# 2thleZ/flash_attention_metal

Measured on AMD Instinct MI355X. Metric: attn_fwd_tflops (seqlen=4096, head_dim=64, bf16, causal), higher is better.
Workload: dtype bf16; 1 GPU; BASELINE.json configs[2]: seqlen=4096 head_dim=64 batch=4 heads=16 bf16 is_causal=true per GPU; batch_per_gpu=4, heads=16, seq_len=4096, head_dim=64, is_causal=True

## Files before the change

### flash_attention_metal_amd/csrc/fa_api.hip

```cpp
#include <stdarg.h>
#include <algorithm>
#include <initializer_list>
#include <stdio.h>
#include <string.h>

#include "fa_common.h"

namespace {
thread_local char g_err[512] = "";

int fail(int code, const char *fmt, ...) {
  va_list ap;
  va_start(ap, fmt);
  vsnprintf(g_err, sizeof(g_err), fmt, ap);
  va_end(ap);
  return code;
}

#define TRY(check) do { if (const int st_ = (check)) return st_; } while (0)

int nonnull(const char *fn, std::initializer_list<const void *> ptrs) {
  for (const void *p : ptrs)
    if (!p) return fail(FA_ERR_INVALID_ARG, "%s: null pointer", fn);
  return FA_OK;
// ... 84 lines not shown
  return e == hipSuccess ? FA_OK : fail(FA_ERR_LAUNCH, "%s: launch failed: %s", fn, hipGetErrorString(e));
}
}

extern "C" {

const char *fa_last_error(void) { return g_err; }
int fa_version(void) { return FA_MI355_VERSION; }

const char *fa_variant_name(int v) {
  switch (v) {
    case FA_VARIANT_AUTO: return "auto";
    case FA_VARIANT_NAIVE: return "naive";
    case FA_VARIANT_TILED: return "tiled";
    case FA_VARIANT_TILED_V2: return "tiled_v2";
    case FA_VARIANT_MFMA: return "mfma";
    case FA_VARIANT_MFMA_PP: return "mfma_pp";
    case FA_VARIANT_MFMA_SPLITKV: return "mfma_splitkv";
    case FA_VARIANT_MFMA_SPLIT2: return "mfma_split2";
    case FA_VARIANT_MFMA_EXACT: return "mfma_exact";
    case FA_VARIANT_MFMA_H64S2: return "mfma_h64s2";
    case FA_VARIANT_MFMA16: return "mfma16";
    case FA_VARIANT_MFMA_FP8PV: return "mfma_fp8pv";
    default: return "?";
  }
}
const char *fa_dtype_name(int d) {
  switch (d) {
    case FA_DTYPE_F32: return "f32";
    case FA_DTYPE_F16: return "f16";
    case FA_DTYPE_BF16: return "bf16";
    case FA_DTYPE_FP8_E4M3: return "fp8_e4m3";
    default: return "?";
  }
}
int fa_dtype_in_bytes(int d) {
  switch (d) {
    case FA_DTYPE_F32: return 4;
    case FA_DTYPE_F16: case FA_DTYPE_BF16: return 2;
    case FA_DTYPE_FP8_E4M3: return 1;
    default: return 0;
  }
}
int fa_dtype_out_bytes(int d) { return d == FA_DTYPE_FP8_E4M3 ? 2 : fa_dtype_in_bytes(d); }

int fa_supported(int dtype, int variant, int D) {
  switch (variant) {
    case FA_VARIANT_AUTO: return fa_resolve_variant(dtype, D) > 0;
    case FA_VARIANT_NAIVE: return fa::naive_supported(dtype, D);
    case FA_VARIANT_TILED: return fa::tiled_supported(dtype, D);
    case FA_VARIANT_TILED_V2: return fa::tiled_v2_supported(dtype, D);
    case FA_VARIANT_MFMA: return fa::mfma_supported(dtype, D);
    case FA_VARIANT_MFMA_PP: return 0;
    case FA_VARIANT_MFMA_SPLITKV: return fa::splitkv_supported(dtype, D);
    case FA_VARIANT_MFMA_SPLIT2: return fa::mfma_split2_supported(dtype, D);
    case FA_VARIANT_MFMA_EXACT: return fa::mfma_supported(dtype, D);
    case FA_VARIANT_MFMA_H64S2: return fa::mfma_h64s2_supported(dtype, D);
    case FA_VARIANT_MFMA16: return fa::mfma16_supported(dtype, D);
    case FA_VARIANT_MFMA_FP8PV: return fa::fp8pv_supported(dtype, D);
    default: return 0;
  }
}
int fa_resolve_variant(int dtype, int D) {
  if (fa::mfma_supported(dtype, D)) return FA_VARIANT_MFMA;
  if (fa::mfma16_supported(dtype, D)) return FA_VARIANT_MFMA16;
  if (fa::tiled_v2_supported(dtype, D)) return FA_VARIANT_TILED_V2;
  return FA_ERR_UNSUPPORTED;
}

static int route_auto(int dtype, int D, int B, int H, int Nq, int Nk, int is_causal, bool ex) {
  const long long blocks128 = (long long)B * H * ((Nq + 127) / 128);
  if (D == 64 && fa::splitkv_supported(dtype, D) && Nk > 64 && blocks128 <= 64) return FA_VARIANT_MFMA_SPLITKV;
  const int v = fa_resolve_variant(dtype, D);
  if (v != FA_VARIANT_MFMA) return v;
  if (ex)
    return fa::mfma16_supported(dtype, D) && blocks128 > 512 && Nk >= (D == 64 ? (is_causal ? 1536 : 1024) : (is_causal ? 2048 : 1024))
               ? FA_VARIANT_MFMA16
               : FA_VARIANT_MFMA;
  const int N = Nq;
  const long long blocks64 = (long long)B * H * ((N + 63) / 64);
  if (fa::mfma_h64s2_supported(dtype, D) && N >= 256 && blocks64 <= 512) return FA_VARIANT_MFMA_H64S2;
  const bool fp8_d128 = dtype == FA_DTYPE_FP8_E4M3 && D == 128;
// ... 42 lines not shown
double fa_algorithmic_bytes(int B, int H, int N, int D, int dtype) {
  return (3.0 * fa_dtype_in_bytes(dtype) + fa_dtype_out_bytes(dtype)) * (double)B * H * N * D +
         4.0 * (double)B * H * N;
}

static hipError_t launch_fwd(const void *q, const void *k, const void *v, void *o, float *lse, int B, int Hq, int Hkv, int Nq, int Nk,
                             int D, float scale, long long q_batch_stride, long long q_head_stride, long long kv_batch_stride,
                             long long kv_head_stride, int is_causal, int dtype, int variant, hipStream_t s) {
  fa::Params p;
  p.q = q; p.k = k; p.v = v; p.o = o; p.lse = lse;
  p.B = B; p.H = Hq; p.N = Nq; p.D = D; p.scale = scale;
  p.batch_stride = q_batch_stride; p.head_stride = q_head_stride;
  p.is_causal = is_causal ? 1 : 0;
  p.Nk = Nk; p.Hkv = Hkv; p.kv_batch_stride = kv_batch_stride; p.kv_head_stride = kv_head_stride;
  p.exact = (variant == FA_VARIANT_MFMA_EXACT);
  switch (variant) {
    case FA_VARIANT_NAIVE: return fa::launch_naive(p, dtype, s);
    case FA_VARIANT_TILED: return fa::launch_tiled(p, dtype, s);
    case FA_VARIANT_TILED_V2: return fa::launch_tiled_v2(p, dtype, s);
    case FA_VARIANT_MFMA_SPLITKV: return fa::launch_splitkv(p, dtype, s);
    case FA_VARIANT_MFMA_SPLIT2: return fa::launch_mfma_split2(p, dtype, s);
    case FA_VARIANT_MFMA_H64S2: return fa::launch_mfma_h64s2(p, dtype, s);
    case FA_VARIANT_MFMA16: return fa::launch_mfma16(p, dtype, s);
    case FA_VARIANT_MFMA_FP8PV: return fa::launch_fp8pv(p, dtype, s);
    default: return fa::launch_mfma(p, dtype, s);
  }
}

int fa_fwd(const void *q, const void *k, const void *v, void *o, float *lse, int B, int H, int N,
           int D, float scale, long long batch_stride, long long head_stride, int is_causal,
           int dtype, int variant, void *hip_stream) {
  g_err[0] = 0;
  const char *fn = "fa_fwd";
  TRY(nonnull(fn, {q, k, v, o}));
  TRY(positive(fn, {B, H, N, D}));
  TRY(scale_ok(fn, scale));
  if (fa_dtype_in_bytes(dtype) == 0) return fail(FA_ERR_INVALID_ARG, "fa_fwd: bad dtype %d", dtype);
  TRY(strides_ok(fn, "", N, D, batch_stride, head_stride, stride_mult(dtype), H > 1));
  TRY(aligned16(fn, "tensors", {q, k, v, o}));
  TRY(head_fits(fn, (double)(N + 128) * D * fa_dtype_in_bytes(dtype), 4, ""));
  if (!fa::mfma_supported(dtype, D) && fa::mfma16_supported(dtype, D))
    TRY(head_fits(fn, (double)(N + 128) * D * 2, 2, " (head dims on padded rows)"));
  TRY(grid_fits(fn, (long long)B * H, N));
  if (variant == FA_VARIANT_AUTO) {
    variant = route_auto(dtype, D, B, H, N, N, is_causal, false);
    if (variant < 0)
// ... 20 lines not shown
}

int fa_fwd_exv(const void *q, const void *k, const void *v, void *o, float *lse, int B, int Hq, int Hkv, int Nq, int Nk,
               int D, float scale, long long q_batch_stride, long long q_head_stride, long long kv_batch_stride,
               long long kv_head_stride, int is_causal, int dtype, int variant, void *hip_stream) {
  g_err[0] = 0;
  const char *fn = "fa_fwd_ex";
  TRY(nonnull(fn, {q, k, v, o}));
  TRY(positive(fn, {B, Hq, Hkv, Nq, Nk, D}));
  TRY(grouped(fn, Hq, Hkv));
  TRY(causal_fits(fn, is_causal, Nq, Nk));
  TRY(scale_ok(fn, scale));
  const bool padded_dim = !fa::mfma_supported(dtype, D) && fa::mfma16_supported(dtype, D);
  if (!fa::mfma_supported(dtype, D) && !padded_dim)
    return fail(FA_ERR_UNSUPPORTED, "fa_fwd_ex: needs a matrix-core kernel (f16/bf16: D a multiple of 8 up to 128, or 256; fp8: D=64|128|256), got dtype=%s D=%d",
                fa_dtype_name(dtype), D);
  if (padded_dim) TRY(head_fits(fn, (double)(std::max(Nq, Nk) + 128) * D * 2, 2, " (head dims on padded rows)"));
  TRY(strides_ok(fn, "", Nq, D, q_batch_stride, q_head_stride, stride_mult(dtype), Hq > 1 && B > 1));
  TRY(strides_ok(fn, "key/value ", Nk, D, kv_batch_stride, kv_head_stride, stride_mult(dtype), Hkv > 1 && B > 1));
  TRY(aligned16(fn, "tensors", {q, k, v, o}));
  TRY(head_fits(fn, (double)(std::max(Nq, Nk) + 128) * D * fa_dtype_in_bytes(dtype), 4, ""));
  TRY(grid_fits(fn, (long long)B * Hq, Nq));
  if (variant == FA_VARIANT_AUTO) variant = route_auto(dtype, D, B, Hq, Nq, Nk, is_causal, true);
  if (variant != FA_VARIANT_MFMA && variant != FA_VARIANT_MFMA_EXACT && variant != FA_VARIANT_MFMA16 && variant != FA_VARIANT_MFMA_SPLITKV)
    return fail(FA_ERR_UNSUPPORTED, "fa_fwd_ex: variant=%s does not take grouped heads / Nq != Nk (mfma, mfma_exact, mfma16, mfma_splitkv do)",
                fa_variant_name(variant));
  if (!fa_supported(dtype, variant, D))
    return fail(FA_ERR_UNSUPPORTED, "fa_fwd_ex: variant=%s does not support dtype=%s D=%d", fa_variant_name(variant), fa_dtype_name(dtype), D);
  return launched(fn, launch_fwd(q, k, v, o, lse, B, Hq, Hkv, Nq, Nk, D, scale, q_batch_stride, q_head_stride, kv_batch_stride,
                                 kv_head_stride, is_causal, dtype, variant, (hipStream_t)hip_stream));
}

int fa_fwd_varlen_supported(int dtype, int D) { return fa::mfma_varlen_supported(dtype, D); }
static int varlen_impl(const char *fn, const void *q, const void *k, const void *v, void *o, float *lse, const int *cu_seqlens_q,
                       const int *cu_seqlens_k, int B, int Hq, int Hkv, int total_q, int total_k, int max_seqlen_q, int max_seqlen_k, int D,
                       float scale, long long q_row_stride, long long q_head_stride, long long kv_row_stride, long long kv_head_stride,
                       int window_left, int window_right, int dtype, void *hip_stream, const float *const *sinks = nullptr,
                       const float *softcap = nullptr) {
  g_err[0] = 0;
  TRY(nonnull(fn, {q, k, v, o, cu_seqlens_q, cu_seqlens_k}));
  if (sinks) TRY(sinks_ok(fn, *sinks));
  if (softcap) TRY(softcap_ok(fn, *softcap));
  TRY(positive(fn, {B, Hq, Hkv, total_q, total_k, max_seqlen_q, max_seqlen_k, D}));
  TRY(grouped(fn, Hq, Hkv));
  TRY(scale_ok(fn, scale));
  if (!fa_fwd_varlen_supported(dtype, D))
    return fail(FA_ERR_UNSUPPORTED, "%s: needs f16 / bf16 and D = 64 | 128, got dtype=%s D=%d", fn, fa_dtype_name(dtype), D);
  if (max_seqlen_q > total_q || max_seqlen_k > total_k)
// ... 865 lines not shown
```

### flash_attention_metal_amd/csrc/fa_common.h

```cpp
#pragma once
#include <hip/hip_runtime.h>
#include <stdint.h>

#include <mutex>
#include <set>
#include <utility>

#include "../../include/fa_mi355.h"

namespace fa {

struct FastDiv {
  unsigned mul = 1, sh1 = 0, sh2 = 0;
};
inline FastDiv make_fastdiv(unsigned d) {
  unsigned l = 0;
  while ((1ull << l) < d) ++l;
  FastDiv f;
  f.mul = (unsigned)(((1ull << 32) * ((1ull << l) - d)) / d + 1);
  f.sh1 = l < 1 ? l : 1u;
  f.sh2 = l > 1 ? l - 1 : 0u;
  return f;
}

// ... 173 lines not shown
hipError_t launch_mfma_varlen_paged_sink(const VarlenPagedSinkParams &p, int dtype, hipStream_t s);
hipError_t launch_mfma_varlen_softcap(const VarlenSoftcapParams &p, int dtype, hipStream_t s);
hipError_t launch_mfma_varlen_paged_softcap(const VarlenPagedSoftcapParams &p, int dtype, hipStream_t s);
hipError_t launch_mfma_varlen_paged_kv8(const VarlenPagedSinkParams &p, bool with_sink, hipStream_t s);
bool mfma_varlen_paged_kv8_supported(int q_dtype, int kv_dtype, int D, int page_size);
hipError_t launch_mfma_varlen_paged_ksplit(const VarlenPagedKsplitParams &p, int dtype, hipStream_t s);
int varlen_paged_ksplit_splits(int B, int Hq, int max_seqlen_q, int D, int page_size, int max_pages_per_seq);
struct AppendPagedParams {
  const void *k_new, *v_new;
  void *k_pages, *v_pages;
  const int *cu_new, *block_table, *seqlens;
  int B, Hkv, total_new, max_new, D;
  long long new_rs, new_hs, page_stride, head_stride, row_stride;
  int bt_stride, num_pages, max_pages;
  int lp;
};
constexpr int APPEND_ROWS = 16;
hipError_t launch_kv_append_paged(const AppendPagedParams &p, int elem_bytes, hipStream_t s);
hipError_t launch_kv_append_paged_quant(const AppendPagedParams &p, int new_dtype, float k_mul, float v_mul, hipStream_t s);
hipError_t launch_mfma_split2(const Params &p, int dtype, hipStream_t s);
bool mfma_split2_supported(int dtype, int D);
hipError_t launch_mfma_h64s2(const Params &p, int dtype, hipStream_t s);
bool mfma_h64s2_supported(int dtype, int D);
hipError_t launch_mfma16(const Params &p, int dtype, hipStream_t s);
bool mfma16_supported(int dtype, int D);
int mfma16_waves(int D, int BH, int N, int Nk, int is_causal);
hipError_t launch_fp8pv(const Params &p, int dtype, hipStream_t s);
bool fp8pv_supported(int dtype, int D);
hipError_t launch_splitkv(const Params &p, int dtype, hipStream_t s);

hipError_t launch_decode(const DecodeParams &p, int D, int dtype, int kv8, hipStream_t s);
bool decode_supported(int dtype, int D);
int decode_splits(int B, int Hkv, int Nk, int D, int kv8);
long long decode_workspace_bytes(int B, int Hq, int Hkv, int Nq, int Nk, int D);
hipError_t launch_decode_paged(const DecodePagedParams &p, int D, int dtype, int kv8, hipStream_t s);
hipError_t launch_decode_paged_window(const DecodeWindowParams &p, int D, int dtype, int kv8, hipStream_t s);
hipError_t launch_decode_paged_sink(const DecodeWindowParams &p, const float *sinks, int D, int dtype, int kv8, hipStream_t s);
hipError_t launch_decode_paged_softcap(const DecodeSoftcapParams &p, int D, int dtype, int kv8, hipStream_t s);
hipError_t launch_mla_decode_paged(const MlaDecodeParams &p, int dtype, hipStream_t s);
bool mla_decode_supported(int dtype, int Dqk, int Dv);
int mla_decode_splits(int B, int rblk, int Nk);
long long mla_decode_workspace_bytes(int B, int Hq, int Nq, int Nk);
inline int mla_wide_waves(int rows) { return rows <= 32 ? 2 : 4; }
hipError_t launch_mla_decode_paged_wide(const MlaDecodeParams &p, int dtype, hipStream_t s);
hipError_t launch_mla_combine(const MlaDecodeParams &p, int dtype, hipStream_t s);
long long mla_decode_wide_workspace_bytes(int B, int Hq, int Nq, int Nk);
hipError_t launch_mla_decode_paged_kv8(const MlaDecodeParams &p, hipStream_t s);
long long mla_decode_kv8_workspace_bytes(int B, int Hq, int Nq, int Nk);
// ... 57 lines not shown
```

### flash_attention_metal_amd/csrc/fa_mfma16_kernel.hip

```cpp
#include <stdlib.h>

#include <algorithm>

#include "fa_mfma_common.h"

#ifndef FA16_DEFER_THR
#define FA16_DEFER_THR 8.0f
#endif
#ifndef FA16_LAK
#define FA16_LAK (D == 128 ? 3 : 2)
#endif
#ifndef FA16_LAV
#define FA16_LAV (D == 128 ? 3 : 2)
#endif
#ifndef FA16_PRIO
#define FA16_PRIO 1
#endif
#ifndef FA16_ONES
#define FA16_ONES 1
#endif
#ifndef FA16_LAZY
#define FA16_LAZY 1
#endif
#ifndef FA16_LAZY_THR
#define FA16_LAZY_THR 0x1p20f
// ... 24 lines not shown
#endif
#ifndef FA16_OCC
#define FA16_OCC 4
#endif

namespace fa {

typedef float f32x4 __attribute__((ext_vector_type(4)));

template <typename Tag> struct MT16;
template <> struct MT16<BF16> {
  using elem = __bf16;
  using vec8 = bf16x8;
  __device__ static __forceinline__ f32x4 mfma(vec8 a, vec8 b, f32x4 c) { return __builtin_amdgcn_mfma_f32_16x16x32_bf16(a, b, c, 0, 0, 0); }
};
template <> struct MT16<F16> {
  using elem = _Float16;
  using vec8 = f16x8;
  __device__ static __forceinline__ f32x4 mfma(vec8 a, vec8 b, f32x4 c) { return __builtin_amdgcn_mfma_f32_16x16x32_f16(a, b, c, 0, 0, 0); }
};

__device__ __forceinline__ float xlane(float x, int mask) { return __shfl_xor(x, mask, 64); }

template <typename Tag, int D, int SUB>
constexpr size_t mfma16_lds_bytes() {
  constexpr bool lazy = std::is_same<Tag, BF16>::value && D == 64 && (FA16_ONES != 0) && (FA16_LAZY == 1);
  return 4 * SUB * (size_t)(D == 128 ? FA16_BN128 : BN) * D * 2 + (lazy ? 16 : 0);
}

template <typename Tag, int D, bool CAUSAL, int RW, bool PAD, int SUB>
__device__ __forceinline__ void fwd_mfma16_body(const Params &p) {
  using M = MT16<Tag>;
  using vec8 = typename M::vec8;
  using elem = typename M::elem;
  constexpr int BMR = RW * WM;
  constexpr int RB = D * 2;
  constexpr int CPR = D / 8;
  constexpr int KS = D / 32;
  constexpr int DT = D / 16;
  constexpr int BNK = (D == 128) ? FA16_BN128 : BN;
  constexpr int KT = BNK / 16;
  constexpr int NKP = KT / 2;
  constexpr int TILE = BNK * RB;
  static_assert(D == 64 || D == 128, "head dims of the 16x16x32 kernel");

  extern __shared__ __attribute__((aligned(16))) char smem_generic[];
  lds_char *smem = (lds_char *)smem_generic;
  lds_char *Kbuf = smem;
  lds_char *Vbuf = smem + 2 * SUB * TILE;

  const int wave = __builtin_amdgcn_readfirstlane((int)threadIdx.x >> 6);
  const int lane = threadIdx.x & 63;
  const int c = lane & 15;
  const int g = lane >> 4;

  int bh, qb;
  map_block<CAUSAL>(blockIdx.x, p, bh, qb);
  long long base, base_kv;
  head_bases(bh, p, base, base_kv);
  const int coff = p.Nk - p.N;
  const int q0 = qb * BMR;
  const int qw0 = q0 + wave * WM;

  const int GRB = PAD ? p.D * 2 : RB;
  auto gcol = [&](int chunk) -> unsigned { return (!PAD || chunk * 8 < p.D) ? (unsigned)chunk * 16 : 0x80000000u; };
  const unsigned head_bytes = (unsigned)p.N * GRB, kv_head_bytes = (unsigned)p.Nk * GRB;
  const __amdgpu_buffer_rsrc_t rq = __builtin_amdgcn_make_buffer_rsrc((void *)((const char *)p.q + base * 2), 0, head_bytes, 0x00020000);
  const __amdgpu_buffer_rsrc_t rk = __builtin_amdgcn_make_buffer_rsrc((void *)((const char *)p.k + base_kv * 2), 0, kv_head_bytes, 0x00020000);
  const __amdgpu_buffer_rsrc_t rv = __builtin_amdgcn_make_buffer_rsrc((void *)((const char *)p.v + base_kv * 2), 0, kv_head_bytes, 0x00020000);

  vec8 qf[2][KS];
#pragma unroll
  for (int qt = 0; qt < 2; ++qt)
#pragma unroll
    for (int ks = 0; ks < KS; ++ks) {
      const u32x4 t = __builtin_amdgcn_raw_buffer_load_b128(rq, (unsigned)(qw0 + 16 * qt + c) * GRB + gcol(4 * ks + g), 0, 0);
      qf[qt][ks] = __builtin_bit_cast(vec8, t);
    }

  const int kx = (D == 64) ? ((c >> 1) & 7) : c;
// ... 31 lines not shown
#pragma unroll
    for (int j = 0; j < NPW; ++j) {
      const unsigned soff = PAD ? (unsigned)(t * BNK + j * RW * RPP) * GRB : (unsigned)t * TILE + j * (RW * 1024);
      const unsigned lk = (unsigned)(__UINTPTR_TYPE__)Kbuf + buf * TILE + (wave + RW * j) * 1024;
      const unsigned lv = (unsigned)(__UINTPTR_TYPE__)Vbuf + buf * TILE + (wave + RW * j) * 1024;
      asm volatile("s_mov_b32 m0, %0\n\ts_nop 0\n\tbuffer_load_dwordx4 %1, %2, %3 offen lds" ::"s"(lk), "v"(dma_kvo), "s"(rk), "s"(soff) : "memory");
      asm volatile("s_mov_b32 m0, %0\n\ts_nop 0\n\tbuffer_load_dwordx4 %1, %2, %3 offen lds" ::"s"(lv), "v"(dma_vvo), "s"(rv), "s"(soff) : "memory");
    }
  };

  f32x4 oacc[DT][2];
#pragma unroll
  for (int dt = 0; dt < DT; ++dt)
#pragma unroll
    for (int qt = 0; qt < 2; ++qt)
#pragma unroll
      for (int i = 0; i < 4; ++i) oacc[dt][qt][i] = 0.0f;
  constexpr bool ONES = (FA16_ONES != 0);
  constexpr bool LAZY = ONES && std::is_same<Tag, BF16>::value && D == 64 && (FA16_LAZY != 0);
  constexpr bool LAZY_TEST = LAZY && (FA16_LAZY == 1);
  constexpr bool LOOK_PV = LAZY_TEST && (FA16_LOOK == 1), LOOK_FRONT = LAZY_TEST && (FA16_LOOK == 0);
  constexpr bool COLD3 = LAZY_TEST && (FA16_COLD == 3);
  constexpr bool TAIL_OUT = LAZY_TEST && (FA16_TAIL == 1);
  static_assert(4 * SUB * TILE + (LAZY_TEST ? 4 : 0) <= mfma16_lds_bytes<Tag, D, SUB>() && RW * WM * RB <= 4 * SUB * TILE,
                "the launcher's LDS size covers the K / V buffers, the flag word and the epilogue's O tiles");
  lds_char *poison_flag = smem + 4 * SUB * TILE;
  int slow = 0;
  constexpr float BIAS = !ONES ? 0.0f : std::is_same<Tag, F16>::value ? 3.0f : 7.0f;
  constexpr float FIRST_SUM_FLOOR = std::is_same<Tag, F16>::value ? 1.0f : 0x1p-64f;
  float l[2] = {0.0f, 0.0f};
  f32x4 lacc[2];
#pragma unroll
  for (int qt = 0; qt < 2; ++qt)
#pragma unroll
    for (int i = 0; i < 4; ++i) lacc[qt][i] = 0.0f;
  vec8 ones;
#pragma unroll
  for (int j = 0; j < 8; ++j) ones[j] = (elem)1.0f;
  if constexpr (ONES) asm volatile("" : "+v"(ones));
  const float c2 = p.scale * 1.4426950408889634f;
  f32x4 negm[2];
#pragma unroll
  for (int qt = 0; qt < 2; ++qt) {
#pragma unroll
    for (int i = 0; i < 4; ++i) negm[qt][i] = ONES ? -BIAS : INFINITY;
    asm volatile("" : "+v"(negm[qt]));
  }

  if constexpr (LAZY_TEST) {
    if (threadIdx.x == 0) lds_write_b32(poison_flag, 0u);
  }
  stage_dma(0, 0);
  if constexpr (SUB == 2) {
    if (1 < nT) stage_dma(1, 1);
  }
  asm volatile("s_waitcnt vmcnt(0)" ::: "memory");
#pragma unroll
  for (int qt = 0; qt < 2; ++qt)
#pragma unroll
    for (int ks = 0; ks < KS; ++ks) {
#pragma unroll
      for (int j = 0; j < 8; ++j) qf[qt][ks][j] = (elem)((float)qf[qt][ks][j] * c2);
      asm volatile("" : "+v"(qf[qt][ks]));
    }
  __syncthreads();

  const float sum_thr = __builtin_exp2f(FA16_DEFER_THR);
  auto apply_mask = [&](auto k0c, auto &s, const int kv0) __attribute__((always_inline)) {
    constexpr int K0 = decltype(k0c)::value;
    constexpr int NKT = sizeof(s) / sizeof(s[0]);
    int g4 = 4 * g;
    asm volatile("" : "+v"(g4));
#pragma unroll
    for (int qt = 0; qt < 2; ++qt) {
      int lim = p.Nk - 1 - kv0 - g4;
      if (CAUSAL) lim = min(lim, qw0 + 16 * qt + c + coff - kv0 - g4);
#pragma unroll
      for (int k2 = 0; k2 < NKT; ++k2)
#pragma unroll
// ... 298 lines not shown
            for (int i = 0; i < 4; ++i) {
              lacc[qt][i] = 0.0f;
              negm[qt][i] = -BIAS;
            }
            asm volatile("" : "+v"(negm[qt]));
#pragma unroll
            for (int dt = 0; dt < DT; ++dt)
#pragma unroll
              for (int i = 0; i < 4; ++i) oacc[dt][qt][i] = 0.0f;
          }
          stage_dma(0, 0);
          if constexpr (SUB == 2) {
            if (1 < nT) stage_dma(1, 1);
          }
          asm volatile("s_waitcnt vmcnt(0)" ::: "memory");
          __syncthreads();
          continue;
        }
      }
    }
    break;
  }

  int elane = lane;
  if constexpr (LAZY_TEST) asm volatile("" : "+v"(elane));
  const int ec = elane & 15, eg = elane >> 4;
  lds_char *Ot = smem + wave * (WM * RB);
#pragma unroll
  for (int qt = 0; qt < 2; ++qt) {
    float lt = ONES ? lacc[qt][0] : l[qt];
    if constexpr (!ONES) {
      lt += xlane(lt, 16);
      lt += xlane(lt, 32);
    }
    const float inv_l = __builtin_amdgcn_rcpf(lt);
    const int row = 16 * qt + ec, qrow = qw0 + row;
    if (p.lse != nullptr && eg == 0 && qrow < p.N)
      p.lse[(long long)bh * p.N + qrow] = (__builtin_amdgcn_logf(lt) - negm[qt][0]) * 0.6931471805599453f;
#pragma unroll
    for (int dt = 0; dt < DT; ++dt) {
      typedef elem elem4 __attribute__((ext_vector_type(4)));
      elem4 e;
#pragma unroll
      for (int i = 0; i < 4; ++i) e[i] = (elem)(oacc[dt][qt][i] * inv_l);
      const u32x2 w = __builtin_bit_cast(u32x2, e);
      const int ch = (2 * dt + (eg >> 1)) ^ (row & (CPR - 1));
      lds_write_b64(Ot + row * RB + (ch << 4) + 8 * (eg & 1), w);
    }
  }
  __syncthreads();
  {
    elem *Og = (elem *)p.o + base;
#pragma unroll
    for (int it = 0; it < WM * CPR / 64; ++it) {
      const int idx = it * 64 + elane;
      const int row = idx / CPR, ch = idx % CPR;
      const u32x4 vv = lds_read_b128(Ot + row * RB + ((ch ^ (row & (CPR - 1))) << 4));
      if (qw0 + row < p.N && (!PAD || ch * 8 < p.D)) *reinterpret_cast<u32x4 *>(Og + (long long)(qw0 + row) * (PAD ? p.D : D) + ch * 8) = vv;
    }
  }
}

template <typename Tag, int D, bool CAUSAL, int RW, bool PAD = false, int SUB = 1>
__global__ __launch_bounds__(64 * RW, (D == 64 ? FA16_OCC : FA16_OCC128)) void fwd_mfma16_kernel(Params p) {
  fwd_mfma16_body<Tag, D, CAUSAL, RW, PAD, SUB>(p);
}

bool mfma16_supported(int dtype, int D) { return (dtype == FA_DTYPE_F16 || dtype == FA_DTYPE_BF16) && D >= 8 && D <= 128 && D % 8 == 0; }

template <typename Tag, int D, bool CAUSAL, int RW, bool PAD = false, int SUB = 1>
static hipError_t launch16_one(const Params &p, hipStream_t s) {
  int head_group = causal_head_group(p, D, 2);
#ifdef FA16_FORCE_HEAD_GROUP
  head_group = FA16_FORCE_HEAD_GROUP;
#endif
  return launch_blocks(fwd_mfma16_kernel<Tag, D, CAUSAL, RW, PAD, SUB>, p, RW * WM, 64 * RW, mfma16_lds_bytes<Tag, D, SUB>(), head_group, s);
}

int mfma16_waves(int D, int BH, int N, int Nk, int is_causal) {
#ifdef FA16_FORCE_RW
  return FA16_FORCE_RW;
#endif
  if (D != 64 && D != 128) return 4;
  const long long b256 = (long long)BH * ((N + 255) / 256);
  if (D == 128) return (!is_causal && Nk >= 8192 && b256 >= 1024) ? 8 : 4;
  if (!is_causal) return (Nk >= 512 && b256 >= 512) ? 8 : 4;
  return (Nk >= 4096 && Nk < 6144 && b256 >= 1024 && b256 < 1280) ? 8 : 4;
}

hipError_t launch_mfma16(const Params &p, int dtype, hipStream_t s) {
  const bool w8 = mfma16_waves(p.D, p.B * p.H, p.N, p.Nk, p.is_causal) == 8 && (p.D == 64 || !p.is_causal);
  return with_tag(dtype, [&](auto tag) -> hipError_t {
    using Tag = decltype(tag);
    if (p.D != 64 && p.D != 128) {
      if (p.D < 64) return p.is_causal ? launch16_one<Tag, 64, true, 4, true>(p, s) : launch16_one<Tag, 64, false, 4, true>(p, s);
      return p.is_causal ? launch16_one<Tag, 128, true, 4, true>(p, s) : launch16_one<Tag, 128, false, 4, true>(p, s);
    }
    if (p.D == 64) {
      if (w8) return p.is_causal ? launch16_one<Tag, 64, true, 8, false, FA16_SUB8>(p, s) : launch16_one<Tag, 64, false, 8, false, FA16_SUB8>(p, s);
      return p.is_causal ? launch16_one<Tag, 64, true, 4>(p, s) : launch16_one<Tag, 64, false, 4>(p, s);
    }
    if (p.D == 128) {
      if (w8) return launch16_one<Tag, 128, false, 8>(p, s);
      return p.is_causal ? launch16_one<Tag, 128, true, 4>(p, s) : launch16_one<Tag, 128, false, 4>(p, s);
    }
    return hipErrorInvalidValue;
  });
}

}
```

### flash_attention_metal_amd/ops.py

```python
from __future__ import annotations

import math
from typing import Optional, Tuple

import torch

from ._lib import load_library

DTYPES = {"f32": 0, "f16": 1, "bf16": 2, "fp8_e4m3": 3}
VARIANTS = {"auto": 0, "naive": 1, "tiled": 2, "tiled_v2": 3, "mfma": 4, "mfma_pp": 5, "mfma_splitkv": 6, "mfma_split2": 7, "mfma_exact": 8, "mfma_h64s2": 9, "mfma16": 10, "mfma_fp8pv": 11}

_FP8 = getattr(torch, "float8_e4m3fn", None)
_TORCH2FA = {torch.float32: 0, torch.float16: 1, torch.bfloat16: 2}
if _FP8 is not None:
    _TORCH2FA[_FP8] = 3


class FaError(RuntimeError):
    def __init__(self, status: int, msg: str, entry: str = "fa_fwd"):
        super().__init__(f"{entry} failed ({status}): {msg}")
        self.status = status


def supported(dtype: str, variant: str, D: int) -> bool:
    return bool(load_library().fa_supported(DTYPES[dtype], VARIANTS[variant], D))


def algorithmic_flops(B: int, H: int, N: int, D: int, is_causal: bool) -> float:
    return float(load_library().fa_algorithmic_flops(B, H, N, D, int(is_causal)))


def algorithmic_bytes(B: int, H: int, N: int, D: int, dtype: str) -> float:
    return float(load_library().fa_algorithmic_bytes(B, H, N, D, DTYPES[dtype]))
# ... 894 lines not shown
```

### include/fa_mi355.h

```cpp
#ifndef FA_MI355_H
#define FA_MI355_H

#ifdef __cplusplus
extern "C" {
#endif

#define FA_MI355_VERSION 400

enum fa_dtype {
  FA_DTYPE_F32 = 0,
  FA_DTYPE_F16 = 1,
  FA_DTYPE_BF16 = 2,
  FA_DTYPE_FP8_E4M3 = 3
};

enum fa_variant {
  FA_VARIANT_AUTO = 0,
  FA_VARIANT_NAIVE = 1,
  FA_VARIANT_TILED = 2,
  FA_VARIANT_TILED_V2 = 3,
  FA_VARIANT_MFMA = 4,
  FA_VARIANT_MFMA_PP = 5,
  FA_VARIANT_MFMA_SPLITKV = 6,
  FA_VARIANT_MFMA_SPLIT2 = 7,
  FA_VARIANT_MFMA_EXACT = 8,
  FA_VARIANT_MFMA_H64S2 = 9,
  FA_VARIANT_MFMA16 = 10,
  FA_VARIANT_MFMA_FP8PV = 11
};

enum fa_status {
  FA_OK = 0,
  FA_ERR_INVALID_ARG = -1,
  FA_ERR_UNSUPPORTED = -2,
  FA_ERR_LAUNCH = -3,
  FA_ERR_NO_DEVICE = -4
};

int fa_fwd(const void *q, const void *k, const void *v, void *o, float *lse,
           int B, int H, int N, int D, float scale,
           long long batch_stride, long long head_stride,
           int is_causal, int dtype, int variant, void *hip_stream);

int fa_fwd_ex(const void *q, const void *k, const void *v, void *o, float *lse,
              int B, int Hq, int Hkv, int Nq, int Nk, int D, float scale,
              long long q_batch_stride, long long q_head_stride,
              long long kv_batch_stride, long long kv_head_stride,
              int is_causal, int dtype, void *hip_stream);
int fa_fwd_exv(const void *q, const void *k, const void *v, void *o, float *lse,
               int B, int Hq, int Hkv, int Nq, int Nk, int D, float scale,
               long long q_batch_stride, long long q_head_stride,
// ... 280 lines not shown
```

Baseline: 1160 TFLOP/s.

## Add persistent mfma16 variant with per-XCD ticket scheduling and work stealing

Adds an opt-in persistent-kernel mode for the D=64 mfma16 kernel. A grid sized to the resident block slots pulls query blocks from per-XCD atomic ticket counters and steals from other XCDs' queues once its own queue is empty. This is meant to cut tail imbalance from causal blocks of uneven length. Auto-routing is off by default (FA16_PERSIST_AUTO=0), but the non-persistent D=64 path now also goes through the looped wrapper, reloads kernargs per block, and replaces the epilogue __syncthreads with an lgkmcnt wait, which could change codegen or register pressure.

```diff
diff --git a/flash_attention_metal_amd/csrc/fa_api.hip b/flash_attention_metal_amd/csrc/fa_api.hip
--- a/flash_attention_metal_amd/csrc/fa_api.hip
+++ b/flash_attention_metal_amd/csrc/fa_api.hip
@@ -130,6 +130,7 @@
     case FA_VARIANT_MFMA_H64S2: return "mfma_h64s2";
     case FA_VARIANT_MFMA16: return "mfma16";
     case FA_VARIANT_MFMA_FP8PV: return "mfma_fp8pv";
+    case FA_VARIANT_MFMA16_PERSIST: return "mfma16_persist";
     default: return "?";
   }
 }
@@ -166,6 +167,7 @@
     case FA_VARIANT_MFMA_H64S2: return fa::mfma_h64s2_supported(dtype, D);
     case FA_VARIANT_MFMA16: return fa::mfma16_supported(dtype, D);
     case FA_VARIANT_MFMA_FP8PV: return fa::fp8pv_supported(dtype, D);
+    case FA_VARIANT_MFMA16_PERSIST: return fa::mfma16_persist_supported(dtype, D);
     default: return 0;
   }
 }
@@ -254,6 +256,7 @@
     case FA_VARIANT_MFMA_SPLIT2: return fa::launch_mfma_split2(p, dtype, s);
     case FA_VARIANT_MFMA_H64S2: return fa::launch_mfma_h64s2(p, dtype, s);
     case FA_VARIANT_MFMA16: return fa::launch_mfma16(p, dtype, s);
+    case FA_VARIANT_MFMA16_PERSIST: return fa::launch_mfma16(p, dtype, s, 1);
     case FA_VARIANT_MFMA_FP8PV: return fa::launch_fp8pv(p, dtype, s);
     default: return fa::launch_mfma(p, dtype, s);
   }
@@ -320,8 +323,9 @@
   TRY(head_fits(fn, (double)(std::max(Nq, Nk) + 128) * D * fa_dtype_in_bytes(dtype), 4, ""));
   TRY(grid_fits(fn, (long long)B * Hq, Nq));
   if (variant == FA_VARIANT_AUTO) variant = route_auto(dtype, D, B, Hq, Nq, Nk, is_causal, true);
-  if (variant != FA_VARIANT_MFMA && variant != FA_VARIANT_MFMA_EXACT && variant != FA_VARIANT_MFMA16 && variant != FA_VARIANT_MFMA_SPLITKV)
-    return fail(FA_ERR_UNSUPPORTED, "fa_fwd_ex: variant=%s does not take grouped heads / Nq != Nk (mfma, mfma_exact, mfma16, mfma_splitkv do)",
+  if (variant != FA_VARIANT_MFMA && variant != FA_VARIANT_MFMA_EXACT && variant != FA_VARIANT_MFMA16 && variant != FA_VARIANT_MFMA16_PERSIST &&
+      variant != FA_VARIANT_MFMA_SPLITKV)
+    return fail(FA_ERR_UNSUPPORTED, "fa_fwd_ex: variant=%s does not take grouped heads / Nq != Nk (mfma, mfma_exact, mfma16, mfma16_persist, mfma_splitkv do)",
                 fa_variant_name(variant));
   if (!fa_supported(dtype, variant, D))
     return fail(FA_ERR_UNSUPPORTED, "fa_fwd_ex: variant=%s does not support dtype=%s D=%d", fa_variant_name(variant), fa_dtype_name(dtype), D);
diff --git a/flash_attention_metal_amd/csrc/fa_common.h b/flash_attention_metal_amd/csrc/fa_common.h
--- a/flash_attention_metal_amd/csrc/fa_common.h
+++ b/flash_attention_metal_amd/csrc/fa_common.h
@@ -219,8 +219,10 @@
 bool mfma_split2_supported(int dtype, int D);
 hipError_t launch_mfma_h64s2(const Params &p, int dtype, hipStream_t s);
 bool mfma_h64s2_supported(int dtype, int D);
-hipError_t launch_mfma16(const Params &p, int dtype, hipStream_t s);
+hipError_t launch_mfma16(const Params &p, int dtype, hipStream_t s, int mode = 0);
 bool mfma16_supported(int dtype, int D);
+bool mfma16_persist_supported(int dtype, int D);
+bool mfma16_persist_auto(int D, int BH, int N, int Nk, int is_causal);
 int mfma16_waves(int D, int BH, int N, int Nk, int is_causal);
 hipError_t launch_fp8pv(const Params &p, int dtype, hipStream_t s);
 bool fp8pv_supported(int dtype, int D);
diff --git a/flash_attention_metal_amd/csrc/fa_mfma16_kernel.hip b/flash_attention_metal_amd/csrc/fa_mfma16_kernel.hip
--- a/flash_attention_metal_amd/csrc/fa_mfma16_kernel.hip
+++ b/flash_attention_metal_amd/csrc/fa_mfma16_kernel.hip
@@ -1,6 +1,8 @@
+#include <stdint.h>
 #include <stdlib.h>
 
 #include <algorithm>
+#include <map>
 
 #include "fa_mfma_common.h"
 
@@ -71,14 +73,52 @@
 
 __device__ __forceinline__ float xlane(float x, int mask) { return __shfl_xor(x, mask, 64); }
 
-template <typename Tag, int D, int SUB>
+template <int D, bool PAD>
+constexpr bool mfma16_has_persist() {
+  return D == 64 && !PAD;
+}
+template <typename Tag, int D, int SUB, bool PAD = false>
 constexpr size_t mfma16_lds_bytes() {
   constexpr bool lazy = std::is_same<Tag, BF16>::value && D == 64 && (FA16_ONES != 0) && (FA16_LAZY == 1);
-  return 4 * SUB * (size_t)(D == 128 ? FA16_BN128 : BN) * D * 2 + (lazy ? 16 : 0);
-}
-
-template <typename Tag, int D, bool CAUSAL, int RW, bool PAD, int SUB>
-__device__ __forceinline__ void fwd_mfma16_body(const Params &p) {
+  return 4 * SUB * (size_t)(D == 128 ? FA16_BN128 : BN) * D * 2 + ((lazy || mfma16_has_persist<D, PAD>()) ? 16 : 0);
+}
+
+struct Params16 : Params {
+  unsigned *tickets = nullptr;
+  int steal_from = 0;
+};
+
+#ifdef FA16_STAMPS
+constexpr int STAMP_BLOCKS = 16384;
+__device__ unsigned long long fa16_stamps[4 * STAMP_BLOCKS];
+#endif
+
+__device__ __forceinline__ int home_xcd() {
+#ifndef FA16_XCD_FROM_BLOCK_ID
+  unsigned v;
+  asm volatile("s_getreg_b32 %0, hwreg(HW_REG_XCC_ID, 0, 4)" : "=s"(v));
+  return (int)(v & 7u);
+#else
+  return (int)(blockIdx.x & 7u);
+#endif
+}
+
+__device__ __forceinline__ int opaque0() {
+  int z = 0;
+  asm volatile("" : "+s"(z));
+  return z;
+}
+__device__ __forceinline__ bool persist_mode(const Params16 &p) { return ((uintptr_t)p.tickets | (unsigned)opaque0()) != 0; }
+__device__ __forceinline__ bool first_wave() { return __builtin_amdgcn_readfirstlane(((int)threadIdx.x >> 6) + opaque0()) == 0; }
+
+constexpr int CTL_NEXT = 4, CTL_HOME = 8, CTL_DRAWN = 12;
+constexpr int TICKET_LINE = 32;
+constexpr int TICKET_WORDS = 9 * TICKET_LINE;
+__device__ __forceinline__ unsigned lds_read_b32_volatile(const lds_char *a) {
+  return *reinterpret_cast<const volatile __attribute__((address_space(3))) unsigned *>(a);
+}
+template <typename Tag, int D, bool CAUSAL, int RW, bool PAD, int SUB, bool LOOPED>
+__device__ __forceinline__ void fwd_mfma16_body(const Params16 &p, const int id) {
   using M = MT16<Tag>;
   using vec8 = typename M::vec8;
   using elem = typename M::elem;
@@ -99,12 +139,23 @@
   lds_char *Vbuf = smem + 2 * SUB * TILE;
 
   const int wave = __builtin_amdgcn_readfirstlane((int)threadIdx.x >> 6);
-  const int lane = threadIdx.x & 63;
+  int lane_id = threadIdx.x & 63;
+  if constexpr (LOOPED) asm volatile("" : "+v"(lane_id));
+  const int lane = lane_id;
   const int c = lane & 15;
   const int g = lane >> 4;
 
+#ifdef FA16_STAMPS
+  const unsigned long long stamp_entry = __builtin_amdgcn_s_memrealtime();
+#endif
+  unsigned ticket = 0;
+  if constexpr (LOOPED) {
+    if (persist_mode(p) && threadIdx.x == 0 && lds_read_b32_volatile((lds_char *)smem_generic + 4 * SUB * TILE + CTL_HOME) != 0)
+      ticket = __hip_atomic_fetch_add(p.tickets + TICKET_LINE * home_xcd(), 1u, __ATOMIC_RELAXED, __HIP_MEMORY_SCOPE_AGENT);
+  }
+
   int bh, qb;
-  map_block<CAUSAL>(blockIdx.x, p, bh, qb);
+  map_block<CAUSAL>(id, p, bh, qb);
   long long base, base_kv;
   head_bases(bh, p, base, base_kv);
   const int coff = p.Nk - p.N;
@@ -182,7 +233,7 @@
   constexpr bool LOOK_PV = LAZY_TEST && (FA16_LOOK == 1), LOOK_FRONT = LAZY_TEST && (FA16_LOOK == 0);
   constexpr bool COLD3 = LAZY_TEST && (FA16_COLD == 3);
   constexpr bool TAIL_OUT = LAZY_TEST && (FA16_TAIL == 1);
-  static_assert(4 * SUB * TILE + (LAZY_TEST ? 4 : 0) <= mfma16_lds_bytes<Tag, D, SUB>() && RW * WM * RB <= 4 * SUB * TILE,
+  static_assert(4 * SUB * TILE + (LAZY_TEST ? 4 : 0) + (LOOPED ? 12 : 0) <= mfma16_lds_bytes<Tag, D, SUB, PAD>() && RW * WM * RB <= 4 * SUB * TILE,
                 "the launcher's LDS size covers the K / V buffers, the flag word and the epilogue's O tiles");
   lds_char *poison_flag = smem + 4 * SUB * TILE;
   int slow = 0;
@@ -215,6 +266,10 @@
     if (1 < nT) stage_dma(1, 1);
   }
   asm volatile("s_waitcnt vmcnt(0)" ::: "memory");
+  if constexpr (LOOPED) {
+    asm volatile("" : "+v"(ticket));
+    if (persist_mode(p) && threadIdx.x == 0) lds_write_b32((lds_char *)smem_generic + 4 * SUB * TILE + CTL_DRAWN, ticket);
+  }
 #pragma unroll
   for (int qt = 0; qt < 2; ++qt)
 #pragma unroll
@@ -559,8 +614,8 @@
     break;
   }
 
-  int elane = lane;
-  if constexpr (LAZY_TEST) asm volatile("" : "+v"(elane));
+  int elane = LOOPED ? (int)(threadIdx.x & 63) : lane;
+  if constexpr (LAZY_TEST || LOOPED) asm volatile("" : "+v"(elane));
   const int ec = elane & 15, eg = elane >> 4;
   lds_char *Ot = smem + wave * (WM * RB);
 #pragma unroll
@@ -585,7 +640,7 @@
       lds_write_b64(Ot + row * RB + (ch << 4) + 8 * (eg & 1), w);
     }
   }
-  __syncthreads();
+  asm volatile("s_waitcnt lgkmcnt(0)" ::: "memory");
   {
     elem *Og = (elem *)p.o + base;
 #pragma unroll
@@ -596,22 +651,229 @@
       if (qw0 + row < p.N && (!PAD || ch * 8 < p.D)) *reinterpret_cast<u32x4 *>(Og + (long long)(qw0 + row) * (PAD ? p.D : D) + ch * 8) = vv;
     }
   }
+#ifdef FA16_STAMPS
+  asm volatile("s_waitcnt vmcnt(0)" ::: "memory");
+  if (threadIdx.x == 0 && id < STAMP_BLOCKS) {
+    fa16_stamps[4 * id + 0] = stamp_entry;
+    fa16_stamps[4 * id + 1] = __builtin_amdgcn_s_memrealtime();
+    fa16_stamps[4 * id + 2] = ((unsigned long long)blockIdx.x << 8) | (unsigned)home_xcd();
+    fa16_stamps[4 * id + 3] = (unsigned long long)nT;
+  }
+#endif
+}
+
+template <bool CAUSAL, int RW, int D>
+__device__ __forceinline__ int mfma16_block_tiles(const Params16 &p, const int id) {
+  constexpr int BNK = (D == 128) ? FA16_BN128 : BN;
+  int bh, qb;
+  map_block<CAUSAL>(id, p, bh, qb);
+  const int kv_end = CAUSAL ? min(p.Nk, (qb + 1) * RW * WM + p.Nk - p.N) : p.Nk;
+  return (kv_end + BNK - 1) / BNK;
+}
+
+template <bool CAUSAL, int RW, int D>
+__device__ __forceinline__ int mfma16_steal(const Params16 &p, const int total) {
+  int lane = threadIdx.x & 63;
+  asm volatile("" : "+v"(lane));
+  const int l = lane & 7;
+  const int len = total > l ? (total - l + 7) >> 3 : 0;
+  for (int attempt = 0; attempt < 8; ++attempt) {
+    const unsigned seen = __hip_atomic_load(p.tickets + TICKET_LINE * l, __ATOMIC_RELAXED, __HIP_MEMORY_SCOPE_AGENT);
+    const int left = seen < (unsigned)len ? len - (int)seen : 0;
+    int key = 0;
+    if (left > 0)
+      key = (mfma16_block_tiles<CAUSAL, RW, D>(p, 8 * (int)seen + l) < p.steal_from ? 1 << 30 : 0) | (min(left, (1 << 26) - 1) << 3) | l;
+    key = max(key, __shfl_xor(key, 1, 64));
+    key = max(key, __shfl_xor(key, 2, 64));
+    key = max(key, __shfl_xor(key, 4, 64));
+    key = __builtin_amdgcn_readfirstlane(key);
+    if (key == 0) return -1;
+    const int v = key & 7;
+    unsigned t = 0;
+    if (lane == 0) t = __hip_atomic_fetch_add(p.tickets + TICKET_LINE * v, 1u, __ATOMIC_RELAXED, __HIP_MEMORY_SCOPE_AGENT);
+    t = (unsigned)__builtin_amdgcn_readfirstlane((int)t);
+    if (t < (unsigned)((total - v + 7) >> 3)) return 8 * (int)t + v;
+  }
+  return -1;
+}
+
+template <bool CAUSAL, int RW, int D>
+__device__ __forceinline__ void mfma16_next_block(const Params16 &p, lds_char *ctl) {
+  const int total = ((p.nq + opaque0()) * p.B + opaque0()) * p.H;
+  const int x = home_xcd();
+  const int len_home = total > x ? (total - x + 7) >> 3 : 0;
+  const int home = __builtin_amdgcn_readfirstlane((int)lds_read_b32_volatile(ctl + CTL_HOME));
+  const unsigned drawn = (unsigned)__builtin_amdgcn_readfirstlane((int)lds_read_b32_volatile(ctl + CTL_DRAWN));
+  int next;
+  if (home != 0 && drawn < (unsigned)len_home) {
+    next = 8 * (int)drawn + x;
+  } else {
+    if (home != 0 && threadIdx.x == 0) lds_write_b32(ctl + CTL_HOME, 0u);
+    next = mfma16_steal<CAUSAL, RW, D>(p, total);
+  }
+  if (threadIdx.x == 0) lds_write_b32(ctl + CTL_NEXT, (unsigned)next);
+}
+
+template <typename Tag, int D, bool CAUSAL, int RW, bool PAD, int SUB>
+__device__ __forceinline__ void fwd_mfma16_blocks(const Params16 &p) {
+  extern __shared__ __attribute__((aligned(16))) char smem_generic[];
+  constexpr int BNK = (D == 128) ? FA16_BN128 : BN;
+  lds_char *ctl = (lds_char *)smem_generic + 4 * SUB * BNK * D * 2;
+  int id = blockIdx.x;
+  if (persist_mode(p) && first_wave()) {
+    unsigned t = 0;
+    if (threadIdx.x == 0) {
+      t = __hip_atomic_fetch_add(p.tickets + TICKET_LINE * home_xcd(), 1u, __ATOMIC_RELAXED, __HIP_MEMORY_SCOPE_AGENT);
+      lds_write_b32(ctl + CTL_HOME, 1u);
+      lds_write_b32(ctl + CTL_DRAWN, t);
+    }
+  }
+  for (;;) {
+    if (persist_mode(p)) {
+      if (first_wave()) mfma16_next_block<CAUSAL, RW, D>(p, ctl);
+      __syncthreads();
+      id = __builtin_amdgcn_readfirstlane((int)lds_read_b32_volatile(ctl + CTL_NEXT));
+      if (id < 0) break;
+    }
+    {
+      typedef const __attribute__((address_space(4))) unsigned *kernarg_words;
+      kernarg_words args = (kernarg_words)__builtin_amdgcn_kernarg_segment_ptr();
+      asm volatile("" : "+s"(args));
+      Params16 pb;
+      static_assert(sizeof(pb) % 4 == 0, "copied by words");
+#pragma unroll
+      for (unsigned i = 0; i < sizeof(pb) / 4; ++i) reinterpret_cast<u32_alias *>(&pb)[i] = args[i];
+      fwd_mfma16_body<Tag, D, CAUSAL, RW, PAD, SUB, true>(pb, id);
+    }
+    if (!persist_mode(p)) return;
+  }
+  if (first_wave()) {
+    unsigned done = 0;
+    if (threadIdx.x == 0) done = __hip_atomic_fetch_add(p.tickets + TICKET_LINE * 8, 1u, __ATOMIC_RELAXED, __HIP_MEMORY_SCOPE_AGENT);
+    if ((unsigned)__builtin_amdgcn_readfirstlane((int)done) == gridDim.x - 1u && (threadIdx.x & 63) < 9)
+      __hip_atomic_store(p.tickets + TICKET_LINE * (threadIdx.x & 63), 0u, __ATOMIC_RELAXED, __HIP_MEMORY_SCOPE_AGENT);
+  }
 }
 
 template <typename Tag, int D, bool CAUSAL, int RW, bool PAD = false, int SUB = 1>
-__global__ __launch_bounds__(64 * RW, (D == 64 ? FA16_OCC : FA16_OCC128)) void fwd_mfma16_kernel(Params p) {
-  fwd_mfma16_body<Tag, D, CAUSAL, RW, PAD, SUB>(p);
+__global__ __launch_bounds__(64 * RW, (D == 64 ? FA16_OCC : FA16_OCC128)) void fwd_mfma16_kernel(Params16 p) {
+  if constexpr (mfma16_has_persist<D, PAD>()) fwd_mfma16_blocks<Tag, D, CAUSAL, RW, PAD, SUB>(p);
+  else fwd_mfma16_body<Tag, D, CAUSAL, RW, PAD, SUB, false>(p, blockIdx.x);
 }
 
 bool mfma16_supported(int dtype, int D) { return (dtype == FA_DTYPE_F16 || dtype == FA_DTYPE_BF16) && D >= 8 && D <= 128 && D % 8 == 0; }
+bool mfma16_persist_supported(int dtype, int D) { return (dtype == FA_DTYPE_F16 || dtype == FA_DTYPE_BF16) && D == 64; }
+
+constexpr int PERSIST_SETS = 1024;
+struct TicketTable {
+  unsigned *base = nullptr;
+  int used = 0;
+  hipStream_t owner[PERSIST_SETS];
+};
+static hipError_t ticket_set_for(hipStream_t s, unsigned **set) {
+  static std::mutex mu;
+  static TicketTable tables[16];
+  int dev = 0;
+  hipError_t e = hipGetDevice(&dev);
+  if (e != hipSuccess) return e;
+  if (dev < 0 || dev >= 16) return hipErrorInvalidDevice;
+  hipStreamCaptureStatus cap = hipStreamCaptureStatusNone;
+  if (s != nullptr && hipStreamIsCapturing(s, &cap) != hipSuccess) {
+    (void)hipGetLastError();
+    cap = hipStreamCaptureStatusNone;
+  }
+  std::lock_guard<std::mutex> g(mu);
+  TicketTable &t = tables[dev];
+  if (t.base == nullptr) {
+    hipStreamCaptureMode mode = hipStreamCaptureModeRelaxed;
+    (void)hipThreadExchangeStreamCaptureMode(&mode);
+    unsigned *b = nullptr;
+    e = hipMalloc((void **)&b, (size_t)PERSIST_SETS * TICKET_WORDS * sizeof(unsigned));
+    if (e == hipSuccess) e = hipMemset(b, 0, (size_t)PERSIST_SETS * TICKET_WORDS * sizeof(unsigned));
+    if (e == hipSuccess) e = hipDeviceSynchronize();
+    (void)hipThreadExchangeStreamCaptureMode(&mode);
+    if (e != hipSuccess) {
+      if (b != nullptr) (void)hipFree(b);
+      return e;
+    }
+    t.base = b;
+  }
+  int idx = -1;
+  if (cap == hipStreamCaptureStatusNone)
+    for (int i = 0; i < t.used && idx < 0; ++i)
+      if (t.owner[i] == s) idx = i;
+  if (idx < 0) {
+    if (t.used == PERSIST_SETS) return hipErrorOutOfMemory;
+    idx = t.used++;
+    t.owner[idx] = cap == hipStreamCaptureStatusNone ? s : (hipStream_t)(uintptr_t)-1;
+  }
+  *set = t.base + (size_t)idx * TICKET_WORDS;
+  return hipSuccess;
+}
+
+static hipError_t resident_slots(const void *kern, int threads, size_t lds, int *slots) {
+  static std::mutex mu;
+  static std::map<std::pair<const void *, int>, int> known;
+  int dev = 0;
+  hipError_t e = hipGetDevice(&dev);
+  if (e != hipSuccess) return e;
+  std::lock_guard<std::mutex> g(mu);
+  auto it = known.find({kern, dev});
+  if (it == known.end()) {
+    int per_cu = 0, cus = 0;
+    e = hipOccupancyMaxActiveBlocksPerMultiprocessor(&per_cu, kern, threads, lds);
+    if (e == hipSuccess) e = hipDeviceGetAttribute(&cus, hipDeviceAttributeMultiprocessorCount, dev);
+    if (e != hipSuccess) return e;
+    if (per_cu < 1 || cus < 1) return hipErrorInvalidValue;
+    it = known.insert({{kern, dev}, per_cu * cus}).first;
+  }
+  *slots = it->second;
+  return hipSuccess;
+}
+
+#ifndef FA16_STEAL_FROM
+#define FA16_STEAL_FROM 68
+#endif
+static int mfma16_steal_from() {
+  const char *e = getenv("FA_MI355_STEAL_FROM");
+  return (e != nullptr && *e != 0) ? atoi(e) : FA16_STEAL_FROM;
+}
+static int mfma16_grid_cap() {
+  const char *e = getenv("FA_MI355_PERSIST_GRID");
+  const int v = (e != nullptr && *e != 0) ? atoi(e) : 0;
+  return v > 0 ? v : 0x7fffffff;
+}
 
 template <typename Tag, int D, bool CAUSAL, int RW, bool PAD = false, int SUB = 1>
-static hipError_t launch16_one(const Params &p, hipStream_t s) {
+static hipError_t launch16_one(const Params &p, hipStream_t s, bool persist = false) {
   int head_group = causal_head_group(p, D, 2);
 #ifdef FA16_FORCE_HEAD_GROUP
   head_group = FA16_FORCE_HEAD_GROUP;
 #endif
-  return launch_blocks(fwd_mfma16_kernel<Tag, D, CAUSAL, RW, PAD, SUB>, p, RW * WM, 64 * RW, mfma16_lds_bytes<Tag, D, SUB>(), head_group, s);
+  Params16 pp;
+  static_cast<Params &>(pp) = p;
+  auto kern = fwd_mfma16_kernel<Tag, D, CAUSAL, RW, PAD, SUB>;
+  constexpr size_t lds = mfma16_lds_bytes<Tag, D, SUB, PAD>();
+  if constexpr (mfma16_has_persist<D, PAD>()) {
+    if (persist) {
+      const int nQ = (p.N + RW * WM - 1) / (RW * WM);
+      const long long total = (long long)nQ * p.B * p.H;
+      if (total > 0x7fffffffLL) return hipErrorInvalidValue;
+      hipError_t e = lds > 48 * 1024 ? set_dyn_lds_once((const void *)kern, (int)lds) : hipSuccess;
+      int slots = 0;
+      if (e == hipSuccess) e = resident_slots((const void *)kern, 64 * RW, lds, &slots);
+      if (e == hipSuccess) e = ticket_set_for(s, &pp.tickets);
+      if (e != hipSuccess) return e;
+      pp.steal_from = mfma16_steal_from();
+      pp.head_group = head_group;
+      set_block_divisors(pp, nQ, head_group);
+      (void)hipGetLastError();
+      hipLaunchKernelGGL(kern, dim3((unsigned)std::min<long long>(std::min(slots, mfma16_grid_cap()), total)), dim3(64 * RW), lds, s, pp);
+      return hipGetLastError();
+    }
+  }
+  if (persist) return hipErrorInvalidValue;
+  return launch_blocks(kern, pp, RW * WM, 64 * RW, lds, head_group, s);
 }
 
 int mfma16_waves(int D, int BH, int N, int Nk, int is_causal) {
@@ -625,8 +887,25 @@
   return (Nk >= 4096 && Nk < 6144 && b256 >= 1024 && b256 < 1280) ? 8 : 4;
 }
 
-hipError_t launch_mfma16(const Params &p, int dtype, hipStream_t s) {
+#ifndef FA16_PERSIST_AUTO
+#define FA16_PERSIST_AUTO 0
+#endif
+bool mfma16_persist_auto(int D, int BH, int N, int Nk, int is_causal) {
+#ifdef FA16_FORCE_PERSIST
+  return FA16_FORCE_PERSIST != 0 && D == 64;
+#endif
+  return FA16_PERSIST_AUTO != 0 && D == 64 && is_causal != 0 && mfma16_waves(D, BH, N, Nk, is_causal) == 8;
+}
+
+hipError_t launch_mfma16(const Params &p, int dtype, hipStream_t s, int mode) {
   const bool w8 = mfma16_waves(p.D, p.B * p.H, p.N, p.Nk, p.is_causal) == 8 && (p.D == 64 || !p.is_causal);
+  if (mode == 1 && p.D != 64) return hipErrorInvalidValue;
+  if (mode == 0 && mfma16_persist_auto(p.D, p.B * p.H, p.N, p.Nk, p.is_causal)) {
+    const hipError_t e = launch_mfma16(p, dtype, s, 1);
+    if (e != hipErrorOutOfMemory) return e;
+    (void)hipGetLastError();
+  }
+  const bool persist = mode == 1;
   return with_tag(dtype, [&](auto tag) -> hipError_t {
     using Tag = decltype(tag);
     if (p.D != 64 && p.D != 128) {
@@ -634,8 +913,8 @@
       return p.is_causal ? launch16_one<Tag, 128, true, 4, true>(p, s) : launch16_one<Tag, 128, false, 4, true>(p, s);
     }
     if (p.D == 64) {
-      if (w8) return p.is_causal ? launch16_one<Tag, 64, true, 8, false, FA16_SUB8>(p, s) : launch16_one<Tag, 64, false, 8, false, FA16_SUB8>(p, s);
-      return p.is_causal ? launch16_one<Tag, 64, true, 4>(p, s) : launch16_one<Tag, 64, false, 4>(p, s);
+      if (w8) return p.is_causal ? launch16_one<Tag, 64, true, 8, false, FA16_SUB8>(p, s, persist) : launch16_one<Tag, 64, false, 8, false, FA16_SUB8>(p, s, persist);
+      return p.is_causal ? launch16_one<Tag, 64, true, 4>(p, s, persist) : launch16_one<Tag, 64, false, 4>(p, s, persist);
     }
     if (p.D == 128) {
       if (w8) return launch16_one<Tag, 128, false, 8>(p, s);
@@ -646,3 +925,14 @@
 }
 
 }
+
+#ifdef FA16_STAMPS
+extern "C" int fa16_debug_read_stamps(void *dst, long long bytes) {
+  if (bytes > (long long)sizeof(unsigned long long) * 4 * fa::STAMP_BLOCKS) return -1;
+  if (hipDeviceSynchronize() != hipSuccess) return -2;
+  if (hipMemcpyFromSymbol(dst, HIP_SYMBOL(fa::fa16_stamps), (size_t)bytes) != hipSuccess) return -3;
+  void *dev = nullptr;
+  if (hipGetSymbolAddress(&dev, HIP_SYMBOL(fa::fa16_stamps)) != hipSuccess) return -4;
+  return hipMemset(dev, 0, sizeof(unsigned long long) * 4 * fa::STAMP_BLOCKS) == hipSuccess ? 0 : -5;
+}
+#endif
diff --git a/flash_attention_metal_amd/ops.py b/flash_attention_metal_amd/ops.py
--- a/flash_attention_metal_amd/ops.py
+++ b/flash_attention_metal_amd/ops.py
@@ -8,7 +8,8 @@
 from ._lib import load_library
 
 DTYPES = {"f32": 0, "f16": 1, "bf16": 2, "fp8_e4m3": 3}
-VARIANTS = {"auto": 0, "naive": 1, "tiled": 2, "tiled_v2": 3, "mfma": 4, "mfma_pp": 5, "mfma_splitkv": 6, "mfma_split2": 7, "mfma_exact": 8, "mfma_h64s2": 9, "mfma16": 10, "mfma_fp8pv": 11}
+VARIANTS = {"auto": 0, "naive": 1, "tiled": 2, "tiled_v2": 3, "mfma": 4, "mfma_pp": 5, "mfma_splitkv": 6, "mfma_split2": 7, "mfma_exact": 8, "mfma_h64s2": 9, "mfma16": 10, "mfma_fp8pv": 11,
+            "mfma16_persist": 12}
 
 _FP8 = getattr(torch, "float8_e4m3fn", None)
 _TORCH2FA = {torch.float32: 0, torch.float16: 1, torch.bfloat16: 2}
diff --git a/include/fa_mi355.h b/include/fa_mi355.h
--- a/include/fa_mi355.h
+++ b/include/fa_mi355.h
@@ -26,7 +26,8 @@
   FA_VARIANT_MFMA_EXACT = 8,
   FA_VARIANT_MFMA_H64S2 = 9,
   FA_VARIANT_MFMA16 = 10,
-  FA_VARIANT_MFMA_FP8PV = 11
+  FA_VARIANT_MFMA_FP8PV = 11,
+  FA_VARIANT_MFMA16_PERSIST = 12
 };
 
 enum fa_status {
```

Result: slower. 1134 TFLOP/s (-2.3%).
